# 0xC0000054/avif-format

Hardware: NVIDIA H100
Metric: Gpixels/s (higher is better)
Workload: dtype f32

## Files before the change

avif-format_b200/csrc/kernels_fast_flat.cu:

```cuda
#include "kernels_fast_common.cuh"
#include "table_staging.cuh"
#include "../../include/avifgpu.h"

namespace avifgpu
{

using namespace avifpix;
using namespace fastenc;
using namespace staging;
using avifmath::LibmTables;

namespace
{

#ifndef AVIF_FLAT_WARPS
#define AVIF_FLAT_WARPS 28
#endif
constexpr int kFlatWarps = AVIF_FLAT_WARPS;
constexpr int kFlatThreads = kFlatWarps * 32;
constexpr int kRowSegmentBytes = kTilePixels * 12;
constexpr int kStageBytesPerWarp = 2 * kRowSegmentBytes;
constexpr int kRowSegmentWords = kRowSegmentBytes / 4;
constexpr int kSharedBarriers = 256;
constexpr int kTableBarrierSlot = kSharedBarriers / 8 - 1;
static_assert(kFlatWarps <= kTableBarrierSlot, "the warps' barriers and the table's share kSharedBarriers");
constexpr int kSharedLimit = 227 * 1024;
__host__ __device__ constexpr int FlatFixedBytes() { return kSharedLibm + kSharedBarriers + kFlatWarps * kStageBytesPerWarp; }

struct FlatSchedule
{
    int32_t tilesX, tileRows, warpCount;
    int32_t segments, items;
    int32_t segmentRows, longSegments;
    int32_t lastColumnBytes;
    int32_t unpairedTileRow;
    int32_t scatter;
};

__device__ __forceinline__ bool ElectOne()
{
    uint32_t elected;
    asm volatile("{ .reg .pred p; elect.sync _|p, 0xffffffff; selp.u32 %0, 1, 0, p; }" : "=r"(elected));
    return elected != 0;
}

template <int CURVE, int XS, int YS, int TWO_LEVEL, int INTERLEAVED>
__global__ void __launch_bounds__(kFlatThreads, 1) EncodeRgbF32FlatKernel(const FastEncodeParams p, const FlatSchedule schedule)
{
    constexpr bool kCompact = TWO_LEVEL >= 2;
    constexpr int kCompactShift = TWO_LEVEL == 3 ? 14 : 0;
    extern __shared__ __align__(128) uint8_t sharedBytes[];
    uint64_t* libmStorage = reinterpret_cast<uint64_t*>(sharedBytes);
    uint64_t* barriers = reinterpret_cast<uint64_t*>(sharedBytes + kSharedLibm);
    uint8_t* stageAll = sharedBytes + kSharedLibm + kSharedBarriers;
    uint2* flatEntries = reinterpret_cast<uint2*>(sharedBytes + FlatFixedBytes());
    uint32_t* compactEntries = reinterpret_cast<uint32_t*>(sharedBytes + FlatFixedBytes());
    const uint32_t* firstBits = compactEntries + ((p.table.flatCount + 3) & ~3);
    uint2* octaves = reinterpret_cast<uint2*>(sharedBytes + FlatFixedBytes());
    uint32_t* bucketWords = reinterpret_cast<uint32_t*>(sharedBytes + FlatFixedBytes() + 2048);

    const int lane = threadIdx.x & 31;
    const int warpInBlock = __shfl_sync(0xffffffffu, static_cast<int>(threadIdx.x >> 5), 0);
    const uint32_t barrier = SharedAddress(barriers + warpInBlock);
    uint32_t* stage = reinterpret_cast<uint32_t*>(stageAll + warpInBlock * kStageBytesPerWarp);
    const uint32_t stageAddress = SharedAddress(stage);
    const uint32_t* myStage = stage + lane * 12;

    const int tilesX = schedule.tilesX;
    const int warpCount = schedule.warpCount;
    const int firstItem = schedule.scatter ? warpInBlock * static_cast<int>(gridDim.x) + static_cast<int>(blockIdx.x) : static_cast<int>(blockIdx.x) * kFlatWarps + warpInBlock;
    constexpr int kChromaRowsPerTile = YS ? 1 : 2;
    constexpr int kChromaTileBytes = XS ? kTilePixels : 2 * kTilePixels;

    auto itemRows = [&](int item, int& column, int& rowBegin, int& rowEnd)
    {
        const int segment = item / tilesX;
        column = item - segment * tilesX;
        rowBegin = segment * schedule.segmentRows + min(segment, schedule.longSegments);
        rowEnd = rowBegin + schedule.segmentRows + (segment < schedule.longSegments ? 1 : 0);
    };
    auto fetchTile = [&](int row, uint32_t bytes, int64_t offset)
    {
        const bool second = row != schedule.unpairedTileRow;
        const uint8_t* source = p.rows + offset;
        BarrierExpect(barrier, second ? 2u * bytes : bytes);
        BulkCopyToShared(stageAddress, source, bytes, barrier);
        if (second)
        {
            BulkCopyToShared(stageAddress + kRowSegmentBytes, source + p.rowStride, bytes, barrier);
        }
    };
    auto columnBytes = [&](int column) { return column == tilesX - 1 ? static_cast<uint32_t>(schedule.lastColumnBytes) : static_cast<uint32_t>(kRowSegmentBytes); };
    auto sourceOffsetOf = [&](int row, int column) { return static_cast<int64_t>(row) * 2 * p.rowStride + static_cast<int64_t>(column) * kRowSegmentBytes; };

    if (kCompact && threadIdx.x == 0)
    {
        BeginTableImageCopy(p.table, compactEntries, barriers + kTableBarrierSlot);
    }
    if (ElectOne())
    {
        BarrierInit(barrier, 1);
        BarrierInitFence();
        if (firstItem < schedule.items)
        {
            int column, rowBegin, rowEnd;
            itemRows(firstItem, column, rowBegin, rowEnd);
            if (rowBegin < rowEnd)
            {
                fetchTile(rowBegin, columnBytes(column), sourceOffsetOf(rowBegin, column));
            }
        }
    }

    const LibmTables t = avifmath::StageLibmTables(libmStorage, threadIdx.x, blockDim.x);
    if (kCompact)
    {
    }
    else if (TWO_LEVEL)
    {
        for (int i = threadIdx.x; i < 256; i += blockDim.x)
        {
            octaves[i] = p.table.octaves[i];
        }
        for (int i = threadIdx.x; i < p.table.bucketCount; i += blockDim.x)
        {
            bucketWords[i] = p.table.buckets[i];
        }
    }
    else
    {
        const uint4* source = reinterpret_cast<const uint4*>(p.table.flat);
        uint4* target = reinterpret_cast<uint4*>(flatEntries);
        const int pairs = (p.table.flatCount + 1) / 2;
#pragma unroll 8
        for (int i = threadIdx.x; i < pairs; i += blockDim.x)
        {
            target[i] = __ldg(source + i);
        }
    }
    __syncthreads();
    if (kCompact)
    {
        WaitTableImage(barriers + kTableBarrierSlot);
    }

    const uint32_t flatShift = p.table.flatShift;
    const int32_t negativeLow = -static_cast<int32_t>(p.table.flatLow);
    const int32_t span = static_cast<int32_t>(p.table.flatHigh - p.table.flatLow);
    const uint32_t bandStrideLog2 = p.table.bandStrideLog2;
    const uint32_t* __restrict__ bandBits = p.table.bandBits;
    const uint32_t compactTopShift = 32u - flatShift;
    const uint32_t compactCodeMask = p.table.compactCodeMask;
    const uint32_t compactMagic = p.table.compactMagic;
    uint32_t parity = 0;

#pragma unroll 1
    for (int item = firstItem; item < schedule.items; item += warpCount)
    {
        int column, rowBegin, rowEnd;
        itemRows(item, column, rowBegin, rowEnd);
        if (item != firstItem && rowBegin < rowEnd && ElectOne())
        {
            fetchTile(rowBegin, columnBytes(column), sourceOffsetOf(rowBegin, column));
        }
        const uint32_t tileBytes = columnBytes(column);
        const bool laneActive = column * kTilePixels + lane * 4 < p.width;
        int64_t sourceOffset = sourceOffsetOf(rowBegin, column);
        uint8_t* yPointer = p.planeY + static_cast<int64_t>(rowBegin) * 2 * p.strideY +
                            (INTERLEAVED ? static_cast<int64_t>(column) * (6 * kTilePixels) + lane * 24 : static_cast<int64_t>(column) * (2 * kTilePixels) + lane * 8);
        uint8_t* cbPointer = p.planeCb + static_cast<int64_t>(rowBegin) * kChromaRowsPerTile * p.strideCb + static_cast<int64_t>(column) * kChromaTileBytes + lane * (XS ? 4 : 8);
        uint8_t* crPointer = p.planeCr + static_cast<int64_t>(rowBegin) * kChromaRowsPerTile * p.strideCr + static_cast<int64_t>(column) * kChromaTileBytes + lane * (XS ? 4 : 8);

#pragma unroll 1
    for (int tileRow = rowBegin; tileRow < rowEnd; ++tileRow)
    {
        const bool secondRow = tileRow != schedule.unpairedTileRow;
        sourceOffset += 2 * p.rowStride;

        BarrierWait(barrier, parity);
        parity ^= 1u;

        float codeF[kValuesPerLane];
        uint32_t bandMask = 0;
        int32_t largest = 0;
#pragma unroll
        for (int q = 0; q < 6; ++q)
        {
            const uint4 w = *reinterpret_cast<const uint4*>(myStage + (q / 3) * kRowSegmentWords + (q % 3) * 4);
            const uint32_t bits[4] = { w.x, w.y, w.z, w.w };
#pragma unroll
            for (int e = 0; e < 4; ++e)
            {
                const int j = 4 * q + e;
                bool inBand;
                if (kCompact)
                {
                    uint32_t entry;
                    codeF[j] = LookupCurveCompact<kCompactShift>(bits[e], compactEntries, flatShift, negativeLow, span, compactTopShift, compactCodeMask,
                                                                 compactMagic, inBand, entry);
                }
                else if (TWO_LEVEL)
                {
                    codeF[j] = CodeToFloat(LookupCurveCode(bits[e], octaves, bucketWords, inBand));
                }
                else
                {
                    codeF[j] = LookupCurveFlat(bits[e], flatEntries, flatShift, negativeLow, span, inBand);
                }
                asm("{ .reg .pred p; setp.ne.u32 p, %1, 0; @p or.b32 %0, %0, %2; }" : "+r"(bandMask) : "r"(static_cast<uint32_t>(inBand)), "r"(1u << j));
            }
            if (TWO_LEVEL != 1)
            {
                largest = max(largest, __vimax3_s32(static_cast<int32_t>(w.x), static_cast<int32_t>(w.y), static_cast<int32_t>(w.z)));
                largest = max(largest, static_cast<int32_t>(w.w));
            }
        }

        auto stagedBits = [&](int j) { return myStage[j + (j >= 12 ? kRowSegmentWords - 12 : 0)]; };
        uint32_t lowerMask = 0;
        if (kCompact)
        {
            uint32_t pending = bandMask;
            while (pending != 0)
            {
                uint32_t word[2] = { 0xffffffffu, 0xffffffffu }, index[2] = { 0u, 0u }, sampleBit[2] = { 0u, 0u };
#pragma unroll
                for (int u = 0; u < 2; ++u)
                {
                    if (pending != 0)
                    {
                        const int j = __ffs(static_cast<int>(pending)) - 1;
                        pending &= pending - 1;
                        const uint32_t bits = stagedBits(j);
                        const int32_t bucket = __viaddmin_s32_relu(static_cast<int32_t>(bits) >> flatShift, negativeLow, span);
                        const uint32_t entry = compactEntries[bucket];
                        const uint32_t k = ((entry & compactCodeMask) >> kCompactLenBits) + ((entry >> compactTopShift) != 0 ? 1u : 0u);
                        const uint32_t distance = bits - firstBits[k];
                        if (k != 0 && distance < (1u << bandStrideLog2))
                        {
                            index[u] = (k << bandStrideLog2) + distance;
                            word[u] = __ldg(bandBits + (index[u] >> 5));
                            sampleBit[u] = 1u << j;
                        }
                    }
                }
#pragma unroll
                for (int u = 0; u < 2; ++u)
                {
                    if (((word[u] >> (index[u] & 31u)) & 1u) == 0)
                    {
                        lowerMask |= sampleBit[u];
                    }
                }
            }
        }
        else if (!TWO_LEVEL)
        {
            uint32_t pending = bandMask;
            while (pending != 0)
            {
                const int j0 = __ffs(static_cast<int>(pending)) - 1;
                pending &= pending - 1;
                const uint32_t bits0 = stagedBits(j0);
                bool inBand;
                uint2 entry0;
                LookupCurveFlat(bits0, flatEntries, flatShift, negativeLow, span, inBand, entry0);
                const uint32_t index0 = BandBitIndex(bits0, entry0, bandStrideLog2);
                const uint32_t word0 = __ldg(bandBits + (index0 >> 5));
                uint32_t word1 = 0xffffffffu, index1 = 0, sample1 = 0;
                if (pending != 0)
                {
                    const int j1 = __ffs(static_cast<int>(pending)) - 1;
                    pending &= pending - 1;
                    const uint32_t bits1 = stagedBits(j1);
                    uint2 entry1;
                    LookupCurveFlat(bits1, flatEntries, flatShift, negativeLow, span, inBand, entry1);
                    index1 = BandBitIndex(bits1, entry1, bandStrideLog2);
                    word1 = __ldg(bandBits + (index1 >> 5));
                    sample1 = 1u << j1;
                }
                lowerMask |= (((word0 >> (index0 & 31u)) & 1u) ^ 1u) << j0;
                if (((word1 >> (index1 & 31u)) & 1u) == 0)
                {
                    lowerMask |= sample1;
                }
            }
        }

        if (__any_sync(0xffffffffu, TWO_LEVEL == 1 ? bandMask != 0 : largest > 0x7f7fffff))
        {
            for (int j = 0; j < kValuesPerLane; ++j)
            {
                const uint32_t bits = stagedBits(j);
                if (TWO_LEVEL == 1 ? ((bandMask >> j) & 1u) != 0 : static_cast<int32_t>(bits) > 0x7f7fffff)
                {
                    const float exact = CodeToFloat(ExactCurveCode<CURVE>(__uint_as_float(bits), p.pqMultiplier, p.maxCodeFloat, t));
#pragma unroll
                    for (int slot = 0; slot < kValuesPerLane; ++slot)
                    {
                        if (slot == j)
                        {
                            codeF[slot] = exact;
                        }
                    }
                }
            }
        }

        __syncwarp();
        if (tileRow + 1 < rowEnd && ElectOne())
        {
            fetchTile(tileRow + 1, tileBytes, sourceOffset);
        }

#pragma unroll
        for (int j = 0; j < kValuesPerLane; ++j)
        {
            if (lowerMask & (1u << j))
            {
                codeF[j] -= 1.0f;
            }
        }

        if (laneActive)
        {
            if (INTERLEAVED)
            {
#pragma unroll
                for (int r = 0; r < 2; ++r)
                {
                    if (r == 1 && !secondRow) break;
                    uint32_t words[6];
#pragma unroll
                    for (int w = 0; w < 6; ++w)
                    {
                        words[w] = __float2uint_rz(codeF[12 * r + 2 * w]) | (__float2uint_rz(codeF[12 * r + 2 * w + 1]) << 16);
                    }
                    uint2* target = reinterpret_cast<uint2*>(yPointer + r * p.strideY);
                    __stcs(target, make_uint2(words[0], words[1]));
                    __stcs(target + 1, make_uint2(words[2], words[3]));
                    __stcs(target + 2, make_uint2(words[4], words[5]));
                }
            }
            else
            {
                StoreTile<XS, YS>(p, codeF, yPointer, cbPointer, crPointer, secondRow);
            }
        }
        yPointer += 2 * p.strideY;
        cbPointer += kChromaRowsPerTile * p.strideCb;
        crPointer += kChromaRowsPerTile * p.strideCr;
    }
    }
}

inline size_t TableSharedBytes(const FastEncodeParams& fp, int tableKind)
{
    if (tableKind == 1) return 2048 + static_cast<size_t>(fp.table.bucketCount) * sizeof(uint32_t);
    if (tableKind >= 2) return fp.table.compactImageBytes;
    return static_cast<size_t>((fp.table.flatCount + 1) / 2) * sizeof(uint4);
}

template <int CURVE, int XS, int YS, int TWO_LEVEL, int INTERLEAVED = 0>
cudaError_t LaunchFlatKernel(const FastEncodeParams& fp, int smCount, cudaStream_t stream)
{
    const size_t shared = static_cast<size_t>(FlatFixedBytes()) + TableSharedBytes(fp, TWO_LEVEL);
    static std::atomic<uint64_t> configuredDevices{ 0 };
    {
        const cudaError_t e = AllowDynamicShared(EncodeRgbF32FlatKernel<CURVE, XS, YS, TWO_LEVEL, INTERLEAVED>, kSharedLimit, configuredDevices);
        if (e != cudaSuccess)
        {
            return e;
        }
    }
    const long long tiles = static_cast<long long>((fp.width + kTilePixels - 1) / kTilePixels) * ((fp.rowCount + 1) / 2);
    if (tiles > 0x7fffffffll || shared > static_cast<size_t>(kSharedLimit))
    {
        return cudaErrorInvalidValue;
    }
    long long blocks = (tiles + kFlatWarps - 1) / kFlatWarps;
    if (blocks > smCount)
    {
        blocks = smCount;
    }
    FlatSchedule schedule{};
    schedule.tilesX = (fp.width + kTilePixels - 1) / kTilePixels;
    schedule.tileRows = (fp.rowCount + 1) / 2;
    schedule.warpCount = static_cast<int32_t>(blocks) * kFlatWarps;
    schedule.segments = schedule.warpCount / schedule.tilesX;
    if (schedule.segments < 1) schedule.segments = 1;
    if (schedule.segments > schedule.tileRows) schedule.segments = schedule.tileRows;
    schedule.items = schedule.tilesX * schedule.segments;
    schedule.segmentRows = schedule.tileRows / schedule.segments;
    schedule.longSegments = schedule.tileRows % schedule.segments;
    schedule.lastColumnBytes = (fp.width - (schedule.tilesX - 1) * kTilePixels) * 12;
    schedule.unpairedTileRow = (fp.rowCount & 1) ? fp.rowCount / 2 : -1;
    static const bool scatterOff = []() { const char* v = getenv("AVIFGPU_FLAT_SCATTER"); return v != nullptr && v[0] == '0'; }();
    schedule.scatter = scatterOff ? 0 : 1;
    EncodeRgbF32FlatKernel<CURVE, XS, YS, TWO_LEVEL, INTERLEAVED><<<static_cast<unsigned>(blocks), kFlatThreads, shared, stream>>>(fp, schedule);
    return cudaGetLastError();
}

template <int CURVE, int TWO_LEVEL>
cudaError_t DispatchFlatChroma(const FastEncodeParams& fp, int xs, int ys, int smCount, cudaStream_t stream)
{
    if (xs == 1 && ys == 1) return LaunchFlatKernel<CURVE, 1, 1, TWO_LEVEL>(fp, smCount, stream);
    if (xs == 1) return LaunchFlatKernel<CURVE, 1, 0, TWO_LEVEL>(fp, smCount, stream);
    return LaunchFlatKernel<CURVE, 0, 0, TWO_LEVEL>(fp, smCount, stream);
}

}

static bool FlatTableFits(const FastEncodeParams& fp)
{
    return fp.table.flat != nullptr && fp.table.bandBits != nullptr &&
           static_cast<size_t>(FlatFixedBytes()) + TableSharedBytes(fp, 0) <= static_cast<size_t>(kSharedLimit);
}

static bool CompactTableFits(const FastEncodeParams& fp)
{
    return fp.table.compact != nullptr && fp.table.firstBits != nullptr && fp.table.bandBits != nullptr &&
           static_cast<size_t>(FlatFixedBytes()) + TableSharedBytes(fp, 2) <= static_cast<size_t>(kSharedLimit);
}

static bool TwoLevelTableFits(const FastEncodeParams& fp)
{
    return fp.table.buckets != nullptr && fp.table.octaves != nullptr &&
           static_cast<size_t>(FlatFixedBytes()) + TableSharedBytes(fp, 1) <= static_cast<size_t>(kSharedLimit);
}

bool FlatEncodeApplies(const FastEncodeParams& fp)
{
    return CompactTableFits(fp) || FlatTableFits(fp) || TwoLevelTableFits(fp);
}

cudaError_t LaunchFastEncodeFlatInterleaved(const FastEncodeParams& fp, int curve, int smCount, cudaStream_t stream)
{
    if (CompactTableFits(fp))
    {
        if (curve == kCurveLinearToPQ)
        {
            return fp.table.flatShift == 14 ? LaunchFlatKernel<kCurveLinearToPQ, 0, 0, 3, 1>(fp, smCount, stream) : LaunchFlatKernel<kCurveLinearToPQ, 0, 0, 2, 1>(fp, smCount, stream);
        }
        return LaunchFlatKernel<kCurveLinearToSMPTE428, 0, 0, 2, 1>(fp, smCount, stream);
    }
    if (FlatTableFits(fp))
    {
        if (curve == kCurveLinearToPQ) return LaunchFlatKernel<kCurveLinearToPQ, 0, 0, 0, 1>(fp, smCount, stream);
        return LaunchFlatKernel<kCurveLinearToSMPTE428, 0, 0, 0, 1>(fp, smCount, stream);
    }
    if (curve == kCurveLinearToPQ) return LaunchFlatKernel<kCurveLinearToPQ, 0, 0, 1, 1>(fp, smCount, stream);
    return LaunchFlatKernel<kCurveLinearToSMPTE428, 0, 0, 1, 1>(fp, smCount, stream);
}

cudaError_t LaunchFastEncodeFlat(const FastEncodeParams& fp, int curve, int xs, int ys, int smCount, cudaStream_t stream)
{
    if (CompactTableFits(fp) && !fp.preferWideEntries)
    {
        if (curve == kCurveLinearToPQ)
        {
            return fp.table.flatShift == 14 ? DispatchFlatChroma<kCurveLinearToPQ, 3>(fp, xs, ys, smCount, stream) : DispatchFlatChroma<kCurveLinearToPQ, 2>(fp, xs, ys, smCount, stream);
        }
        return DispatchFlatChroma<kCurveLinearToSMPTE428, 2>(fp, xs, ys, smCount, stream);
    }
    if (FlatTableFits(fp))
    {
        if (curve == kCurveLinearToPQ) return DispatchFlatChroma<kCurveLinearToPQ, 0>(fp, xs, ys, smCount, stream);
        return DispatchFlatChroma<kCurveLinearToSMPTE428, 0>(fp, xs, ys, smCount, stream);
    }
    if (curve == kCurveLinearToPQ) return DispatchFlatChroma<kCurveLinearToPQ, 1>(fp, xs, ys, smCount, stream);
    return DispatchFlatChroma<kCurveLinearToSMPTE428, 1>(fp, xs, ys, smCount, stream);
}

}
```

Measured before the change: 184.7.

## Replace static segment schedule with per-CTA tile ranges and shared atomic work counter

```diff
diff --git a/avif-format_b200/csrc/flat_plan.h b/avif-format_b200/csrc/flat_plan.h
--- /dev/null
+++ b/avif-format_b200/csrc/flat_plan.h
@@ -0,0 +1,44 @@
+#ifndef AVIF_FLAT_PLAN_H
+#define AVIF_FLAT_PLAN_H
+
+#include <stdint.h>
+
+#include "kernel_params.h"
+
+namespace avifgpu
+{
+
+AVIFGPU_HD inline int32_t FlatRangeBegin(int32_t cta, int32_t tiles, int32_t ctas)
+{
+    const int32_t base = tiles / ctas;
+    const int32_t longer = tiles % ctas;
+    return cta * base + (cta < longer ? cta : longer);
+}
+
+struct FlatDivider
+{
+    uint64_t multiplier;
+    uint32_t shift;
+};
+
+AVIFGPU_HD inline FlatDivider MakeFlatDivider(uint32_t d)
+{
+    uint32_t l = 0;
+    while ((1ull << l) < d)
+    {
+        ++l;
+    }
+    FlatDivider divider;
+    divider.shift = 31 + l;
+    divider.multiplier = ((1ull << divider.shift) + d - 1) / d;
+    return divider;
+}
+
+AVIFGPU_HD inline int32_t FlatDivide(int32_t n, FlatDivider divider)
+{
+    return static_cast<int32_t>((static_cast<uint64_t>(n) * divider.multiplier) >> divider.shift);
+}
+
+}
+
+#endif
diff --git a/avif-format_b200/csrc/kernels_fast_flat.cu b/avif-format_b200/csrc/kernels_fast_flat.cu
--- a/avif-format_b200/csrc/kernels_fast_flat.cu
+++ b/avif-format_b200/csrc/kernels_fast_flat.cu
@@ -1,6 +1,57 @@
 #include "kernels_fast_common.cuh"
 #include "table_staging.cuh"
+#include "flat_plan.h"
 #include "../../include/avifgpu.h"
+
+#ifdef AVIFGPU_FLAT_TIMELINE
+namespace avifgpu
+{
+constexpr int kTimelineWarps = 6144;
+constexpr int kTimelineTiles = 96;
+struct FlatTimelineWarp
+{
+    uint64_t entry, tableReady, exit;
+    uint32_t smid, warp, tiles, reserved;
+    uint64_t ready[kTimelineTiles];
+    uint64_t stored[kTimelineTiles];
+};
+__device__ FlatTimelineWarp g_flatTimeline[kTimelineWarps];
+__device__ __forceinline__ uint64_t GlobalTimer()
+{
+    uint64_t t;
+    asm volatile("mov.u64 %0, %%globaltimer;" : "=l"(t));
+    return t;
+}
+__device__ __forceinline__ uint32_t SmId()
+{
+    uint32_t id;
+    asm volatile("mov.u32 %0, %%smid;" : "=r"(id));
+    return id;
+}
+inline int32_t TimelineLaunchRecords()
+{
+    static const long long chosen = []() { const char* v = getenv("AVIFGPU_FLAT_TIMELINE_LAUNCH"); return v != nullptr ? atoll(v) : -1ll; }();
+    static std::atomic<long long> launches{ 0 };
+    return launches.fetch_add(1) == chosen ? 1 : 0;
+}
+}
+
+extern "C" AVIFGPU_EXPORT long long avifgpu_flat_timeline_read(void* host, long long bytes)
+{
+    const long long total = static_cast<long long>(sizeof(avifgpu::g_flatTimeline));
+    if (host != nullptr && bytes >= total)
+    {
+        if (cudaDeviceSynchronize() != cudaSuccess || cudaMemcpyFromSymbol(host, avifgpu::g_flatTimeline, total) != cudaSuccess)
+        {
+            return -1;
+        }
+    }
+    return total;
+}
+#define FLAT_TIMELINE(statement) statement
+#else
+#define FLAT_TIMELINE(statement)
+#endif
 
 namespace avifgpu
 {
@@ -21,20 +72,20 @@
 constexpr int kRowSegmentBytes = kTilePixels * 12;
 constexpr int kStageBytesPerWarp = 2 * kRowSegmentBytes;
 constexpr int kRowSegmentWords = kRowSegmentBytes / 4;
-constexpr int kSharedBarriers = 256;
+constexpr int kSharedBarriers = 512;
 constexpr int kTableBarrierSlot = kSharedBarriers / 8 - 1;
-static_assert(kFlatWarps <= kTableBarrierSlot, "the warps' barriers and the table's share kSharedBarriers");
+constexpr int kTileCounterSlot = kSharedBarriers / 8 - 2;
+static_assert(kFlatWarps <= kTileCounterSlot, "the warps' barriers, the tile counter and the table's barrier share kSharedBarriers");
 constexpr int kSharedLimit = 227 * 1024;
 __host__ __device__ constexpr int FlatFixedBytes() { return kSharedLibm + kSharedBarriers + kFlatWarps * kStageBytesPerWarp; }
 
-struct FlatSchedule
-{
-    int32_t tilesX, tileRows, warpCount;
-    int32_t segments, items;
-    int32_t segmentRows, longSegments;
+struct FlatTiles
+{
+    int32_t tiles, tilesX;
+    FlatDivider rowOf;
     int32_t lastColumnBytes;
     int32_t unpairedTileRow;
-    int32_t scatter;
+    FLAT_TIMELINE(int32_t recordTimeline;)
 };
 
 __device__ __forceinline__ bool ElectOne()
@@ -45,7 +96,7 @@
 }
 
 template <int CURVE, int XS, int YS, int TWO_LEVEL, int INTERLEAVED>
-__global__ void __launch_bounds__(kFlatThreads, 1) EncodeRgbF32FlatKernel(const FastEncodeParams p, const FlatSchedule schedule)
+__global__ void __launch_bounds__(kFlatThreads, 1) EncodeRgbF32FlatKernel(const FastEncodeParams p, const FlatTiles plan)
 {
     constexpr bool kCompact = TWO_LEVEL >= 2;
     constexpr int kCompactShift = TWO_LEVEL == 3 ? 14 : 0;
@@ -65,24 +116,25 @@
     uint32_t* stage = reinterpret_cast<uint32_t*>(stageAll + warpInBlock * kStageBytesPerWarp);
     const uint32_t stageAddress = SharedAddress(stage);
     const uint32_t* myStage = stage + lane * 12;
-
-    const int tilesX = schedule.tilesX;
-    const int warpCount = schedule.warpCount;
-    const int firstItem = schedule.scatter ? warpInBlock * static_cast<int>(gridDim.x) + static_cast<int>(blockIdx.x) : static_cast<int>(blockIdx.x) * kFlatWarps + warpInBlock;
+    FLAT_TIMELINE(const int timelineWarp = static_cast<int>(blockIdx.x) * kFlatWarps + warpInBlock;
+                  FlatTimelineWarp* const timeline = plan.recordTimeline && lane == 0 && timelineWarp < kTimelineWarps ? g_flatTimeline + timelineWarp : nullptr;
+                  uint32_t timelineTiles = 0;
+                  if (timeline) { timeline->entry = GlobalTimer(); timeline->smid = SmId(); timeline->warp = timelineWarp; })
+
+    const int tilesX = plan.tilesX;
+    const int rangeEnd = FlatRangeBegin(static_cast<int>(blockIdx.x) + 1, plan.tiles, static_cast<int>(gridDim.x));
+    uint32_t* tileCounter = reinterpret_cast<uint32_t*>(barriers + kTileCounterSlot);
+    int tile = FlatRangeBegin(static_cast<int>(blockIdx.x), plan.tiles, static_cast<int>(gridDim.x)) + warpInBlock;
     constexpr int kChromaRowsPerTile = YS ? 1 : 2;
     constexpr int kChromaTileBytes = XS ? kTilePixels : 2 * kTilePixels;
 
-    auto itemRows = [&](int item, int& column, int& rowBegin, int& rowEnd)
-    {
-        const int segment = item / tilesX;
-        column = item - segment * tilesX;
-        rowBegin = segment * schedule.segmentRows + min(segment, schedule.longSegments);
-        rowEnd = rowBegin + schedule.segmentRows + (segment < schedule.longSegments ? 1 : 0);
-    };
-    auto fetchTile = [&](int row, uint32_t bytes, int64_t offset)
-    {
-        const bool second = row != schedule.unpairedTileRow;
-        const uint8_t* source = p.rows + offset;
+    auto fetchTile = [&](int t)
+    {
+        const int row = FlatDivide(t, plan.rowOf);
+        const int column = t - row * tilesX;
+        const uint32_t bytes = column == tilesX - 1 ? static_cast<uint32_t>(plan.lastColumnBytes) : static_cast<uint32_t>(kRowSegmentBytes);
+        const bool second = row != plan.unpairedTileRow;
+        const uint8_t* source = p.rows + static_cast<int64_t>(row) * 2 * p.rowStride + static_cast<int64_t>(column) * kRowSegmentBytes;
         BarrierExpect(barrier, second ? 2u * bytes : bytes);
         BulkCopyToShared(stageAddress, source, bytes, barrier);
         if (second)
@@ -90,25 +142,22 @@
             BulkCopyToShared(stageAddress + kRowSegmentBytes, source + p.rowStride, bytes, barrier);
         }
     };
-    auto columnBytes = [&](int column) { return column == tilesX - 1 ? static_cast<uint32_t>(schedule.lastColumnBytes) : static_cast<uint32_t>(kRowSegmentBytes); };
-    auto sourceOffsetOf = [&](int row, int column) { return static_cast<int64_t>(row) * 2 * p.rowStride + static_cast<int64_t>(column) * kRowSegmentBytes; };
-
-    if (kCompact && threadIdx.x == 0)
-    {
-        BeginTableImageCopy(p.table, compactEntries, barriers + kTableBarrierSlot);
+
+    if (threadIdx.x == 0)
+    {
+        *tileCounter = static_cast<uint32_t>(tile + kFlatWarps);
+        if (kCompact)
+        {
+            BeginTableImageCopy(p.table, compactEntries, barriers + kTableBarrierSlot);
+        }
     }
     if (ElectOne())
     {
         BarrierInit(barrier, 1);
         BarrierInitFence();
-        if (firstItem < schedule.items)
-        {
-            int column, rowBegin, rowEnd;
-            itemRows(firstItem, column, rowBegin, rowEnd);
-            if (rowBegin < rowEnd)
-            {
-                fetchTile(rowBegin, columnBytes(column), sourceOffsetOf(rowBegin, column));
-            }
+        if (tile < rangeEnd)
+        {
+            fetchTile(tile);
         }
     }
 
@@ -143,6 +192,7 @@
     {
         WaitTableImage(barriers + kTableBarrierSlot);
     }
+    FLAT_TIMELINE(if (timeline) { timeline->tableReady = GlobalTimer(); })
 
     const uint32_t flatShift = p.table.flatShift;
     const int32_t negativeLow = -static_cast<int32_t>(p.table.flatLow);
@@ -155,30 +205,15 @@
     uint32_t parity = 0;
 
 #pragma unroll 1
-    for (int item = firstItem; item < schedule.items; item += warpCount)
-    {
-        int column, rowBegin, rowEnd;
-        itemRows(item, column, rowBegin, rowEnd);
-        if (item != firstItem && rowBegin < rowEnd && ElectOne())
-        {
-            fetchTile(rowBegin, columnBytes(column), sourceOffsetOf(rowBegin, column));
-        }
-        const uint32_t tileBytes = columnBytes(column);
-        const bool laneActive = column * kTilePixels + lane * 4 < p.width;
-        int64_t sourceOffset = sourceOffsetOf(rowBegin, column);
-        uint8_t* yPointer = p.planeY + static_cast<int64_t>(rowBegin) * 2 * p.strideY +
-                            (INTERLEAVED ? static_cast<int64_t>(column) * (6 * kTilePixels) + lane * 24 : static_cast<int64_t>(column) * (2 * kTilePixels) + lane * 8);
-        uint8_t* cbPointer = p.planeCb + static_cast<int64_t>(rowBegin) * kChromaRowsPerTile * p.strideCb + static_cast<int64_t>(column) * kChromaTileBytes + lane * (XS ? 4 : 8);
-        uint8_t* crPointer = p.planeCr + static_cast<int64_t>(rowBegin) * kChromaRowsPerTile * p.strideCr + static_cast<int64_t>(column) * kChromaTileBytes + lane * (XS ? 4 : 8);
-
-#pragma unroll 1
-    for (int tileRow = rowBegin; tileRow < rowEnd; ++tileRow)
-    {
-        const bool secondRow = tileRow != schedule.unpairedTileRow;
-        sourceOffset += 2 * p.rowStride;
+    while (tile < rangeEnd)
+    {
+        const int tileRow = FlatDivide(tile, plan.rowOf);
+        const int column = tile - tileRow * tilesX;
+        const bool secondRow = tileRow != plan.unpairedTileRow;
 
         BarrierWait(barrier, parity);
         parity ^= 1u;
+        FLAT_TIMELINE(if (timeline && timelineTiles < kTimelineTiles) { timeline->ready[timelineTiles] = GlobalTimer(); })
 
         float codeF[kValuesPerLane];
         uint32_t bandMask = 0;
@@ -308,9 +343,15 @@
         }
 
         __syncwarp();
-        if (tileRow + 1 < rowEnd && ElectOne())
-        {
-            fetchTile(tileRow + 1, tileBytes, sourceOffset);
+        int next = 0;
+        if (lane == 0)
+        {
+            next = static_cast<int>(atomicAdd(tileCounter, 1u));
+        }
+        next = __shfl_sync(0xffffffffu, next, 0);
+        if (next < rangeEnd && ElectOne())
+        {
+            fetchTile(next);
         }
 
 #pragma unroll
@@ -322,8 +363,10 @@
             }
         }
 
-        if (laneActive)
-        {
+        if (column * kTilePixels + lane * 4 < p.width)
+        {
+            uint8_t* yPointer = p.planeY + static_cast<int64_t>(tileRow) * 2 * p.strideY +
+                                (INTERLEAVED ? static_cast<int64_t>(column) * (6 * kTilePixels) + lane * 24 : static_cast<int64_t>(column) * (2 * kTilePixels) + lane * 8);
             if (INTERLEAVED)
             {
 #pragma unroll
@@ -344,14 +387,16 @@
             }
             else
             {
+                const int64_t chromaOffset = static_cast<int64_t>(column) * kChromaTileBytes + lane * (XS ? 4 : 8);
+                uint8_t* cbPointer = p.planeCb + static_cast<int64_t>(tileRow) * kChromaRowsPerTile * p.strideCb + chromaOffset;
+                uint8_t* crPointer = p.planeCr + static_cast<int64_t>(tileRow) * kChromaRowsPerTile * p.strideCr + chromaOffset;
                 StoreTile<XS, YS>(p, codeF, yPointer, cbPointer, crPointer, secondRow);
             }
         }
-        yPointer += 2 * p.strideY;
-        cbPointer += kChromaRowsPerTile * p.strideCb;
-        crPointer += kChromaRowsPerTile * p.strideCr;
-    }
-    }
+        FLAT_TIMELINE(if (timeline) { if (timelineTiles < kTimelineTiles) timeline->stored[timelineTiles] = GlobalTimer(); ++timelineTiles; })
+        tile = next;
+    }
+    FLAT_TIMELINE(if (timeline) { timeline->tiles = timelineTiles; timeline->exit = GlobalTimer(); })
 }
 
 inline size_t TableSharedBytes(const FastEncodeParams& fp, int tableKind)
@@ -383,21 +428,14 @@
     {
         blocks = smCount;
     }
-    FlatSchedule schedule{};
-    schedule.tilesX = (fp.width + kTilePixels - 1) / kTilePixels;
-    schedule.tileRows = (fp.rowCount + 1) / 2;
-    schedule.warpCount = static_cast<int32_t>(blocks) * kFlatWarps;
-    schedule.segments = schedule.warpCount / schedule.tilesX;
-    if (schedule.segments < 1) schedule.segments = 1;
-    if (schedule.segments > schedule.tileRows) schedule.segments = schedule.tileRows;
-    schedule.items = schedule.tilesX * schedule.segments;
-    schedule.segmentRows = schedule.tileRows / schedule.segments;
-    schedule.longSegments = schedule.tileRows % schedule.segments;
-    schedule.lastColumnBytes = (fp.width - (schedule.tilesX - 1) * kTilePixels) * 12;
-    schedule.unpairedTileRow = (fp.rowCount & 1) ? fp.rowCount / 2 : -1;
-    static const bool scatterOff = []() { const char* v = getenv("AVIFGPU_FLAT_SCATTER"); return v != nullptr && v[0] == '0'; }();
-    schedule.scatter = scatterOff ? 0 : 1;
-    EncodeRgbF32FlatKernel<CURVE, XS, YS, TWO_LEVEL, INTERLEAVED><<<static_cast<unsigned>(blocks), kFlatThreads, shared, stream>>>(fp, schedule);
+    FlatTiles plan{};
+    plan.tiles = static_cast<int32_t>(tiles);
+    plan.tilesX = (fp.width + kTilePixels - 1) / kTilePixels;
+    plan.rowOf = MakeFlatDivider(static_cast<uint32_t>(plan.tilesX));
+    plan.lastColumnBytes = (fp.width - (plan.tilesX - 1) * kTilePixels) * 12;
+    plan.unpairedTileRow = (fp.rowCount & 1) ? fp.rowCount / 2 : -1;
+    FLAT_TIMELINE(plan.recordTimeline = TimelineLaunchRecords();)
+    EncodeRgbF32FlatKernel<CURVE, XS, YS, TWO_LEVEL, INTERLEAVED><<<static_cast<unsigned>(blocks), kFlatThreads, shared, stream>>>(fp, plan);
     return cudaGetLastError();
 }
 
diff --git a/profiles/measure_flat_timeline.py b/profiles/measure_flat_timeline.py
--- /dev/null
+++ b/profiles/measure_flat_timeline.py
@@ -0,0 +1,139 @@
+#!/usr/bin/env python3
+import argparse
+import json
+import os
+import statistics
+import subprocess
+import sys
+
+import numpy as np
+
+ROOT = os.path.dirname(os.path.dirname(os.path.abspath(__file__)))
+LIB_DIR = os.path.join(ROOT, "avif-format_b200", "lib")
+
+TIMELINE_WARPS, TIMELINE_TILES = 6144, 96
+RECORD = np.dtype([("entry", "<u8"), ("table_ready", "<u8"), ("exit", "<u8"), ("smid", "<u4"), ("warp", "<u4"), ("tiles", "<u4"),
+                   ("reserved", "<u4"), ("ready", "<u8", TIMELINE_TILES), ("stored", "<u8", TIMELINE_TILES)])
+
+
+def child(kind, launches, warmup):
+    sys.path[:0] = [ROOT, os.path.join(ROOT, "avif-format_b200", "python"), os.path.join(ROOT, "tests")]
+    import ctypes as C
+
+    import torch
+
+    import avifgpu
+    import bench
+    from avifgpu import abi
+
+    device = torch.device("cuda", 0)
+    torch.cuda.set_device(device)
+    wl = bench.Workload("c2")
+    if kind == "clip":
+        wl.enc = wl.enc.copy(transfer=abi.TRANSFER_CLIP)
+    gpu = avifgpu.Context(0)
+    run = bench.DeviceRun(torch, avifgpu, gpu, wl, device, 3234)
+    _, per_launch = run.timed(launches, warmup, lambda: torch.cuda.synchronize(device))
+    out = {"kind": kind, "library": avifgpu.LIBRARY_PATH, "median_launch_ms": statistics.median(per_launch),
+           "min_launch_ms": min(per_launch), "launch_ms": per_launch,
+           "device": torch.cuda.get_device_name(device)}
+    if kind == "timeline":
+        read = gpu.lib.avifgpu_flat_timeline_read
+        read.restype, read.argtypes = C.c_longlong, [C.c_void_p, C.c_longlong]
+        records = np.zeros(TIMELINE_WARPS, dtype=RECORD)
+        assert read(None, 0) == records.nbytes, "the record layout differs from kernels_fast_flat.cu"
+        assert read(records.ctypes.data, records.nbytes) == records.nbytes
+        out["timeline"] = analyse(records)
+    gpu.close()
+    print(json.dumps(out))
+
+
+def percentile(values, q):
+    return float(np.percentile(np.asarray(values, dtype=np.float64), q)) if len(values) else None
+
+
+def analyse(records):
+    r = records[records["entry"] != 0]
+    assert len(r), "no warp recorded: AVIFGPU_FLAT_TIMELINE_LAUNCH picked no flat launch"
+    t0 = int(r["entry"].min())
+    us = lambda t: (np.asarray(t, dtype=np.int64) - t0) / 1e3
+    entry, exit_ = us(r["entry"]), us(r["exit"])
+    span = float(exit_.max())
+
+    ramps = []
+    for sm in np.unique(r["smid"]):
+        mine = r[(r["smid"] == sm) & (r["tiles"] > 0)]
+        if len(mine):
+            ramps.append(float(us(mine["ready"][:, 0]).min() - us(r["entry"][r["smid"] == sm]).min()))
+
+    periods, waits = [], []
+    for w in r:
+        n = min(int(w["tiles"]), TIMELINE_TILES)
+        if n == 0:
+            continue
+        ready, stored = w["ready"][:n].astype(np.int64), w["stored"][:n].astype(np.int64)
+        periods.extend((np.diff(ready) / 1e3).tolist())
+        waits.append((ready[0] - int(w["table_ready"])) / 1e3)
+        waits.extend(((ready[1:] - stored[:-1]) / 1e3).tolist())
+
+    edges = sorted([(float(t), 1) for t in entry] + [(float(t), -1) for t in exit_])
+    running, last, below_half = 0, 0.0, 0.0
+    for t, step in edges:
+        if running < len(r) / 2:
+            below_half += t - last
+        running += step
+        last = t
+    stamps = np.unique(np.concatenate([r["entry"], r["exit"], r["ready"][r["ready"] != 0], r["stored"][r["stored"] != 0]]).astype(np.int64))
+    steps = np.diff(stamps)
+    tiles = r["tiles"].astype(int)
+    return {
+        "warps": int(len(r)), "sms": int(len(np.unique(r["smid"]))), "tiles": int(tiles.sum()),
+        "timer_resolution_ns": int(steps[steps > 0].min()) if len(steps) else None,
+        "span_us": span,
+        "ramp_us": {"median": statistics.median(ramps), "max": max(ramps), "what": "per SM: first warp entry -> first tile's barrier return"},
+        "table_ready_us": {"median": float(np.median(us(r["table_ready"]) - entry)), "max": float((us(r["table_ready"]) - entry).max())},
+        "tile_period_us": {"median": percentile(periods, 50), "p90": percentile(periods, 90)},
+        "fetch_wait_us": {"median": percentile(waits, 50), "p90": percentile(waits, 90),
+                          "what": "previous tile's last store (or table ready) -> this tile's barrier return"},
+        "tiles_per_warp": {"min": int(tiles.min()), "max": int(tiles.max())},
+        "tail_us": {"first_exit_to_last_exit": float(exit_.max() - exit_.min()), "below_half_warps_running": below_half,
+                    "below_half_fraction_of_span": below_half / span},
+        "last_entry_us": float(entry.max()),
+    }
+
+
+def main():
+    ap = argparse.ArgumentParser()
+    ap.add_argument("--launches", type=int, default=24, help="timed launches per run (at least 20)")
+    ap.add_argument("--warmup", type=int, default=5)
+    ap.add_argument("--timeline-library", default=os.path.join(LIB_DIR, "libavifgpu_timeline.so"))
+    ap.add_argument("--production-library", default=os.path.join(LIB_DIR, "libavifgpu.so"))
+    ap.add_argument("--out", default=None, help="also write the report here")
+    ap.add_argument("--child", choices=("timeline", "production", "clip"), default=None, help=argparse.SUPPRESS)
+    args = ap.parse_args()
+    if args.child:
+        child(args.child, args.launches, args.warmup)
+        return
+    if args.launches < 20:
+        ap.error("--launches must be at least 20")
+    report = {}
+    for kind, library in (("timeline", args.timeline_library), ("production", args.production_library), ("clip", args.production_library)):
+        env = dict(os.environ, AVIFGPU_LIBRARY=os.path.abspath(library),
+                   AVIFGPU_FLAT_TIMELINE_LAUNCH=str(args.warmup + args.launches // 2))
+        out = subprocess.run([sys.executable, os.path.abspath(__file__), "--child", kind, "--launches", str(args.launches),
+                              "--warmup", str(args.warmup)], env=env, capture_output=True, text=True)
+        if out.returncode != 0:
+            raise SystemExit(f"{kind} run failed:\n{out.stdout[-3000:]}{out.stderr[-3000:]}")
+        report[kind] = json.loads(out.stdout.strip().splitlines()[-1])
+        report[kind].pop("launch_ms")
+    report["instrumentation_cost"] = report["timeline"]["median_launch_ms"] / report["production"]["median_launch_ms"] - 1
+    report["c2_over_clip"] = report["production"]["median_launch_ms"] / report["clip"]["median_launch_ms"]
+    text = json.dumps(report, indent=1)
+    print(text)
+    if args.out:
+        with open(args.out, "w") as f:
+            f.write(text + "\n")
+
+
+if __name__ == "__main__":
+    main()
```

Result: faster. 187.2 (median of 6 runs) (+1.4%).
